# igashov/DiffLinker

Measured on NVIDIA H100. Metric: molecules/sec (T=500 denoising), higher is better.
Workload: dtype f32

## Files before the change

### difflinker_b200/csrc/common.cuh

```cuda
#pragma once
#include <cuda_runtime.h>
#include <stdint.h>

namespace dl {

constexpr int H = 128;
constexpr int MAX_DIN = 32;
constexpr int MAX_XHD = 16;

constexpr int OPT_TANH = 1;
constexpr int OPT_MEAN = 2;
constexpr int OPT_SIN = 4;
constexpr int N_SIN_FREQ = 6;
constexpr int N_SIN_FEAT = 4 * N_SIN_FREQ;
__device__ __forceinline__ float sin_freq(int k) { return __int_as_float(__float_as_int(0x1.aceeap-2f) + (k << 24)); }
__device__ __forceinline__ float sin_arg(float r, int k) { return __fmul_rn(__fsqrt_rn(__fadd_rn(r, 1e-8f)), sin_freq(k)); }
__device__ __forceinline__ float radial_rn(float dx, float dy, float dz) {
  return __fadd_rn(__fadd_rn(__fmul_rn(dx, dx), __fmul_rn(dy, dy)), __fmul_rn(dz, dz));
}

__device__ __forceinline__ void chain_wait() { asm volatile("griddepcontrol.wait;" ::: "memory"); }
__device__ __forceinline__ void chain_release() { asm volatile("griddepcontrol.launch_dependents;" ::: "memory"); }

inline bool& chain_overlap_enabled() { static bool on = true; return on; }

template <typename... KArgs, typename... Args>
inline cudaError_t launch_chain(void (*kernel)(KArgs...), dim3 grid, dim3 block, size_t smem, cudaStream_t st, Args&&... args) {
  cudaLaunchConfig_t cfg = {};
  cfg.gridDim = grid; cfg.blockDim = block; cfg.dynamicSmemBytes = smem; cfg.stream = st;
  cudaLaunchAttribute at[1];
  at[0].id = cudaLaunchAttributeProgrammaticStreamSerialization;
  at[0].val.programmaticStreamSerializationAllowed = chain_overlap_enabled() ? 1 : 0;
  cfg.attrs = at; cfg.numAttrs = 1;
  return cudaLaunchKernelEx(&cfg, kernel, KArgs(static_cast<Args&&>(args))...);
}

__device__ __forceinline__ float silu_f(float x) {
  float t, r;
  asm("ex2.approx.ftz.f32 %0, %1;" : "=f"(t) : "f"(x * -1.4426950408889634f));
// ... 103 lines not shown
```

### difflinker_b200/csrc/dl_engine.cu

```cuda
#include <cuda_fp16.h>
#include <cuda_runtime.h>

#include <algorithm>
#include <cmath>
#include <cstdarg>
#include <cstdio>
#include <cstdlib>
#include <cstring>
#include <ctime>
#include <map>
#include <string>
#include <vector>

#include "../../include/difflinker_b200.h"
#include "kernels_simt.cuh"
#include "kernels_tc.cuh"
#include "kernels_node_tc.cuh"
#include "kernels_retry.cuh"

using namespace dl;

static thread_local char g_err[1024] = "";
static void set_err(const char* fmt, ...) {
  va_list ap;
// ... 424 lines not shown

dl_status enqueue_forward(dl_engine* e, int B, int N, const FwdIO& io, cudaStream_t st) {
  Workspace& ws = e->ws;
  const Geom gm = make_geom(e, B, N);
  const int n = B * N;
  const int L = e->cfg.n_layers, S = e->cfg.inv_sublayers;
  const int node_blocks = (n + NODE_TM - 1) / NODE_TM;
  const size_t node_smem = 3 * NODE_TM * LDX * sizeof(float);

  PrepArgs pa{};
  pa.xh = io.sampler ? ws.z : io.xh;
  pa.node_mask = io.node_mask; pa.linker_mask = io.linker_mask;
  pa.t = io.t; pa.t_numel = io.t_numel; pa.context = io.context;
  pa.We_t = e->We_t; pa.be = e->be; pa.proj = proj_of(e->gcl[0]);
  pa.nm = ws.nm; pa.x0 = ws.x0; pa.x = ws.xa; pa.x04 = e->use_tc ? ws.x04 : nullptr; pa.x4 = e->use_tc ? ws.xa4 : nullptr; pa.cls = ws.cls; pa.h = ws.h;
  pa.AB = e->use_tc ? nullptr : ws.ABg; pa.ABmax = ws.ABgmax;
  pa.coef = io.sampler ? e->coef_dev : nullptr;
  pa.step_prep = io.sampler ? e->step_ctr : nullptr;
  pa.step_fin = io.sampler ? e->step_ctr + 1 : nullptr;
  TIMED("k_prep", st, (launch_chain(k_prep, dim3(node_blocks), dim3(256), 0, st, gm, pa)));
  LAUNCH_CHECK();
  e->launches += 1;
  if (e->use_tc) {
    const tcn::NodeTcArgs ta = node_tc_args(e, e->gcl[0], 0, -1);
    TIMED("k_node_tc(proj only)", st, (tcn::launch_node(n, ta, st)));
    LAUNCH_CHECK();
    e->launches += 1;
  }

  if (ws.nbr != nullptr) {
// ... 22 lines not shown
      if (e->use_tc) {
        const tcn::NodeTcArgs ta = node_tc_args(e, w, l, s);
        TIMED(ta.n_proj == 2 ? "k_node_tc(2 proj)" : "k_node_tc(1 proj)", st, (tcn::launch_node(n, ta, st)));
      } else {
        NodeArgs na{};
        na.h = ws.h; na.agg = ws.agg; na.nm = ws.nm; na.W3_t = w.W3_t; na.b3 = w.b3; na.W4_t = w.W4_t; na.b4 = w.b4;
        NodeConsumer c[2];
        const int n_proj = node_consumers(e, l, s, c);
        na.proj1 = proj_of(*c[0].w); na.AB1 = c[0].AB; na.ABmax1 = c[0].ABmax;
        if (n_proj == 2) { na.proj2 = proj_of(*c[1].w); na.AB2 = c[1].AB; na.ABmax2 = c[1].ABmax; }
        k_node<ACT_SILU><<<node_blocks, 256, node_smem, st>>>(n, na);
      }
      LAUNCH_CHECK();
      e->launches += 1;
    }
    k_copy_x<<<(n * 3 + 255) / 256, 256, 0, st>>>(n * 3, xin, xout, e->use_tc ? xin4 : nullptr, xout4);
    LAUNCH_CHECK();
    e->launches += 1;
    const EqW& w = e->eq[l];
    const EdgeArgs ea = edge_args(e, w, true, io.edge_mask, io.linker_mask, xin, xin4, xout, xout4, w.w5);
    e->times.begin(st, "edge COORD");
    dl_status st2 = launch_edge(e, gm, ea, true, w.W2_tc, st);
    e->times.end(st);
    if (st2 != DL_OK) return st2;
    std::swap(xin, xout);
    std::swap(xin4, xout4);
  }

  FinishArgs fa{};
  fa.h = ws.h; fa.x = xin; fa.x0 = ws.x0; fa.nm = ws.nm; fa.Wo = e->Wo; fa.bo = e->bo;
  fa.nan_flags = io.nan_flags;
  const bool fused_update = io.sampler && !io.inpaint;
  fa.out = fused_update ? nullptr : (io.sampler ? ws.eps : io.out);
// ... 1057 lines not shown
```

### difflinker_b200/csrc/kernels_node_tc.cuh

```cuda
#pragma once
#include "kernels_tc.cuh"

namespace dl {
namespace tcn {

using namespace dl::tc;

constexpr int TM = 128;
constexpr int X_LBO = TM * 16 + 16;
constexpr int X_BYTES = KC * X_LBO;
constexpr int HALF_BYTES = 8 * W_LBO;
constexpr int STAGE_BYTES = 2 * HALF_BYTES;
constexpr int BLOCK_BYTES = 2 * W_BYTES;
constexpr int N_RING = 2;
constexpr int N_OFF_WS = 4 * X_BYTES;
constexpr int N_OFF_MISC = N_OFF_WS + N_RING * STAGE_BYTES;
constexpr int N_OFF_BAR = N_OFF_MISC + 128 * 4 + 64;
constexpr int N_SMEM_BYTES = N_OFF_BAR + 64 + 1024;
static_assert(N_SMEM_BYTES <= 232448, "k_node_tc shared memory");
constexpr int NW = 8;
constexpr int W_NLOADER = NW;
constexpr int NODE_TC_THREADS = 32 * (NW + 1);

struct NodeTcArgs {
// ... 21 lines not shown
    sc = __int_as_float(max(127 + 13 - ex, 1) << 23);
  }
  return sc;
}

__device__ __forceinline__ void workers_sync() { asm volatile("bar.sync 1, %0;" ::"n"(32 * NW) : "memory"); }

__device__ __forceinline__ void store_elem(uint8_t* xhi, uint8_t* xlo, int c, int n, float v) {
  const __half hi = __float2half_rn(v);
  const __half lo = __float2half_rn(v - __half2float(hi));
  const int off = (c >> 3) * X_LBO + n * 16 + (c & 7) * 2;
  *reinterpret_cast<__half*>(xhi + off) = hi;
  *reinterpret_cast<__half*>(xlo + off) = lo;
}

__global__ void __launch_bounds__(NODE_TC_THREADS, 1) k_node_tc(int n_total, NodeTcArgs a) {
  extern __shared__ uint8_t smem_raw[];
  uint8_t* sm = smem_raw + ((1024u - (smem_u32(smem_raw) & 1023u)) & 1023u);
  const uint32_t sbase = smem_u32(sm);
  const int tid = threadIdx.x, warp = tid >> 5, lane = tid & 31;
  const int tile = a.tile_nodes > 0 ? a.tile_nodes : TM;
  const int g0 = blockIdx.x * tile;
  const int n_live = min(tile, n_total - g0);

  const uint32_t bar_full = sbase + N_OFF_BAR, bar_empty = bar_full + 8 * N_RING;
  uint8_t* xa_hi = sm; uint8_t* xa_lo = xa_hi + X_BYTES;
  uint8_t* xb_hi = sm + 2 * X_BYTES; uint8_t* xb_lo = xb_hi + X_BYTES;
  float* nms = reinterpret_cast<float*>(sm + N_OFF_MISC);
  int* tilemax = reinterpret_cast<int*>(sm + N_OFF_MISC + 512);

// ... 34 lines not shown
  const int c0 = 64 * g + 16 * (warp & 3) + (lane >> 2);
  int tm_calls = 0;
  auto tile_max = [&](float mx) -> float {
#pragma unroll
    for (int o = 16; o > 0; o >>= 1) mx = fmaxf(mx, __shfl_xor_sync(0xffffffffu, mx, o));
    int* slot = tilemax + (tm_calls++ & 15);
    if (lane == 0) atomicMax(slot, __float_as_int(mx));
    workers_sync();
    return __int_as_float(*slot);
  };
  auto operand_ready = [&]() {
    fence_proxy_async();
    workers_sync();
  };
  int hb = 0;
  float d[64];
#pragma unroll
  for (int i = 0; i < 64; ++i) d[i] = 0.f;
  auto gemm = [&](const uint8_t* xop, int n_blk_half, bool accumulate) {
    for (int k = 0; k < n_blk_half; ++k, ++hb) {
      const int s = hb % N_RING, hf = hb & 1;
      mbar_wait(bar_full + 8 * s, (hb / N_RING) & 1);
      const uint32_t xh = smem_u32(xop) + (8 * hf) * X_LBO, xl = xh + X_BYTES;
      const uint32_t wh = sbase + N_OFF_WS + s * STAGE_BYTES + g * 1024, wl = wh + HALF_BYTES;
      gemm_3xf16(d, wh, wl, W_LBO, xh, xl, X_LBO, 2 * X_LBO, 4, accumulate || k > 0);
      __syncwarp();
      if (lane == 0) mbar_arrive(bar_empty + 8 * s);
    }
  };

  auto load_rows = [&](float scale) -> float {
    float mx = 0.f;
#pragma unroll 1
// ... 33 lines not shown
    if (s1 == 1.0f) break;
  }
  operand_ready();

  if (a.proj_only) {
    s3 = s1;
  } else {
    gemm(xa_hi, 2, false);
    gemm(xb_hi, 2, true);
    workers_sync();
    const float2 bias3 = make_float2(__ldg(a.b3 + c0), __ldg(a.b3 + c0 + 8));
    const float ds1 = a.w3_descale / s1;
#pragma unroll 1
    for (int pass = 0; pass < 2; ++pass) {
      float mx = 0.f;
#pragma unroll
      for (int j = 0; j < 16; ++j)
#pragma unroll
        for (int u = 0; u < 4; ++u) {
          const float v = fmaf(d[4 * j + u], ds1, (u & 2) ? bias3.y : bias3.x);
          mx = fmaxf(mx, fabsf(v));
          store_elem(xb_hi, xb_lo, c0 + (u & 2) * 4, 8 * j + 2 * q + (u & 1), silu_f(v) * s2);
        }
      if (pass == 1) break;
      s2 = pow2_scale_for(tile_max(mx));
      if (s2 == 1.0f) break;
    }
    operand_ready();
    gemm(xb_hi, 2, false);
    const float2 bias4 = make_float2(__ldg(a.b4 + c0), __ldg(a.b4 + c0 + 8));
    const float ds2 = a.w4_descale / s2;
    float mx = 0.f;
#pragma unroll
    for (int j = 0; j < 16; ++j)
#pragma unroll
      for (int u = 0; u < 4; ++u) {
        const int n = 8 * j + 2 * q + (u & 1), c = c0 + (u & 2) * 4;
        float* hp = a.h + (size_t)(g0 + n) * H + c;
        const float hv = n < n_live ? *hp : 0.f;
        const float o = (hv + fmaf(d[4 * j + u], ds2, (u & 2) ? bias4.y : bias4.x)) * nms[n];
        if (n < n_live) *hp = o;
        mx = fmaxf(mx, fabsf(o));
        d[4 * j + u] = o;
        store_elem(xa_hi, xa_lo, c, n, o);
      }
    s3 = pow2_scale_for(tile_max(mx));
    if (s3 != 1.0f) {
#pragma unroll
      for (int j = 0; j < 16; ++j)
#pragma unroll
        for (int u = 0; u < 4; ++u) store_elem(xa_hi, xa_lo, c0 + (u & 2) * 4, 8 * j + 2 * q + (u & 1), d[4 * j + u] * s3);
    }
    operand_ready();
  }

  for (int p = 0; p < a.n_proj; ++p) {
#pragma unroll 1
    for (int pt = 0; pt < 2; ++pt) {
      gemm(xa_hi, 2, false);
      const float2 bias = pt == 0 ? make_float2(__ldg(a.pb1[p] + c0), __ldg(a.pb1[p] + c0 + 8)) : make_float2(0.f, 0.f);
      float* ab = a.AB[p] + (size_t)g0 * 2 * H + pt * H;
      const float ds = a.p_descale[p] / s3;
      float mx = 0.f;
#pragma unroll
      for (int j = 0; j < 16; ++j)
#pragma unroll
        for (int u = 0; u < 4; ++u) {
          const int n = 8 * j + 2 * q + (u & 1);
          const float o = fmaf(d[4 * j + u], ds, (u & 2) ? bias.y : bias.x);
          if (n < n_live) { ab[(size_t)n * 2 * H + c0 + (u & 2) * 4] = o; mx = fmaxf(mx, fabsf(o)); }
        }
      const float tmx = tile_max(mx);
      if (tid < n_live) a.ABmax[p][(size_t)(g0 + tid) * 2 + pt] = tmx;
    }
  }
}

inline size_t pack_blocks(const std::vector<float>& W, int in_stride, int nblk, std::vector<__half>& blob,
                          float* descale) {
  while (blob.size() % 64) blob.push_back(__float2half(0.f));
// ... 15 lines not shown
          const float v = W[(size_t)c * in_stride + b * H + kc * 8 + u] * scale;
          const __half hi = __float2half_rn(v);
          const __half lo = __float2half_rn(v - __half2float(hi));
          blob[off + b * per + ((size_t)kc * H + c) * 8 + u] = hi;
          blob[off + b * per + (size_t)KC * H * 8 + ((size_t)kc * H + c) * 8 + u] = lo;
        }
  return off;
}

inline int pick_tile_nodes(int n, int num_sms) {
  const int per = (n + num_sms - 1) / std::max(num_sms, 1);
  return std::min(TM, std::max(8, (per + 7) & ~7));
}

inline dl_status configure_node() {
  if (cudaFuncSetAttribute(k_node_tc, cudaFuncAttributeMaxDynamicSharedMemorySize, N_SMEM_BYTES) != cudaSuccess) return DL_ERR_CUDA;
  return DL_OK;
}

inline void launch_node(int n, const NodeTcArgs& ta, cudaStream_t st) {
  const int grid = (n + ta.tile_nodes - 1) / ta.tile_nodes;
  launch_chain(k_node_tc, dim3(grid), dim3(NODE_TC_THREADS), N_SMEM_BYTES, st, n, ta);
}

}
}
```

### difflinker_b200/csrc/kernels_simt.cuh

```cuda
#pragma once
#include <curand_kernel.h>

#include "common.cuh"

namespace dl {

__global__ void k_plan_mol(int N, int graph_type, const int8_t* __restrict__ edge_mask,
                           const int8_t* __restrict__ node_mask, const float* __restrict__ linker_mask,
                           int* __restrict__ rowidx, int* __restrict__ colidx, int* __restrict__ xrowidx,
                           int* __restrict__ nr, int* __restrict__ nc, int* __restrict__ nxr) {
  extern __shared__ int sm_plan[];
  int* rowlive = sm_plan;
  int* collive = sm_plan + N;
  const int b = blockIdx.x;
  const int tid = threadIdx.x, lane = tid & 31, warp = tid >> 5, nwarp = blockDim.x >> 5;
  for (int i = tid; i < N; i += blockDim.x) { rowlive[i] = 0; collive[i] = 0; }
  __syncthreads();
  if ((graph_type == 0 || graph_type == 4) && edge_mask != nullptr) {
    const int8_t* em = edge_mask + (size_t)b * N * N;
    for (int i = warp; i < N; i += nwarp) {
      int any = 0;
      for (int j = lane; j < N; j += 32) {
        int v = em[(size_t)i * N + j];
        if (v != 0) { any = 1; collive[j] = 1; }
// ... 153 lines not shown
struct PrepArgs {
  const float* xh;
  const int8_t* node_mask;
  const float* linker_mask;
  const float* t;
  int t_numel;
  const float* context;
  const float* We_t;
  const float* be;
  ProjW proj;
  float* nm;
  float* x0;
  float* x;
  float4* x04;
  float4* x4;
  int* cls;
  float* h;
  float* AB;
  float* ABmax;
  const float* coef;
  const int* step_prep;
  int* step_fin;
};

__global__ void __launch_bounds__(256) k_prep(Geom gm, PrepArgs a) {
  __shared__ __align__(16) float hs[NODE_TM * LDX];
  __shared__ float hin[NODE_TM][MAX_DIN];
  const int tid = threadIdx.x, lane = tid & 31, warp = tid >> 5;
  const int n_total = gm.B * gm.N;
  const int g0 = blockIdx.x * NODE_TM;
// ... 20 lines not shown
        int cidx = d - (gm.D - gm.C);
        v = a.context[(size_t)g * gm.C + cidx];
      }
    }
    hin[r][d] = v;
  }
  if (tid < NODE_TM) {
    int g = g0 + tid;
    if (g < n_total) {
      float m = (float)a.node_mask[g];
      a.nm[g] = m;
      for (int d = 0; d < 3; ++d) {
        float v = a.xh[(size_t)g * xd + d] * m;
        a.x0[(size_t)g * 3 + d] = v;
        a.x[(size_t)g * 3 + d] = v;
        if (a.x4 != nullptr) {
          reinterpret_cast<float*>(a.x04 + g)[d] = v;
          reinterpret_cast<float*>(a.x4 + g)[d] = v;
        }
      }
      if (gm.graph_type >= 1 && gm.graph_type <= 3) {
        int valid = m != 0.f;
        int pk = a.context[(size_t)g * gm.C + gm.C - 1] != 0.f;
        int fr = a.context[(size_t)g * gm.C + gm.C - 2] != 0.f;
        int lk = a.linker_mask != nullptr ? (a.linker_mask[g] != 0.f) : 0;
        int c = 0;
        if (valid) {
          if (gm.graph_type == 1) c = 1;
          else c = (lk || fr) ? 1 : (pk ? 2 : 3);
        }
        a.cls[g] = c;
      }
    }
// ... 282 lines not shown
  float* w5s = w0s + H;
  float* ems = w5s + H;
  float* cds = ems + ET;
  float* phis = cds + ET * 3;
  __shared__ float xacc[COORD ? 1 : 1];
  (void)xacc;

  const int tid = threadIdx.x, lane = tid & 31, warp = tid >> 5;
  const int N = gm.N;
  for (int idx = tid; idx < H * H / 4; idx += 256)
    reinterpret_cast<float4*>(W2s)[idx] = __ldg(reinterpret_cast<const float4*>(a.W2_t) + idx);
  if (tid < H) {
    b2s[tid] = a.b2[tid]; wds[tid] = a.wd[tid]; w0s[tid] = a.w0[tid];
    w5s[tid] = COORD ? a.w5[tid] : 0.f;
  }
  __syncthreads();

  auto divisor = [&](float cnt) { return !MEAN ? gm.normalization_factor : gm.graph_type == 0 ? (float)N : fmaxf(cnt, 1.f); };
  const int n_work = COORD ? *a.plan.n_xmols : *a.plan.n_items;
  for (int wi = blockIdx.x; wi < n_work; wi += gridDim.x) {
    int b, r_begin, r_count;
    if (COORD) { b = a.plan.xmols[wi]; r_begin = 0; r_count = a.plan.nxr[b]; }
    else { int4 it = a.plan.items[wi]; b = it.x; r_begin = it.y; r_count = it.z; }
    const int nc = a.plan.nc[b];
    const int* rows = (COORD ? a.plan.xrowidx : a.plan.rowidx) + (size_t)b * N;
    const int* cols = a.plan.colidx + (size_t)b * N;
    const size_t gb = (size_t)b * N;
    const int8_t* em_mol = a.edge_mask ? a.edge_mask + gb * N : nullptr;
    int per = nc >= ET ? 1 : ET / nc;
    if (per > MAXR) per = MAXR;
// ... 144 lines not shown
            }
            xrun += s;
            if (c0 + ET >= nc) {
              int i = rows[r_begin + rt + rr];
              float lm = a.linker_mask ? a.linker_mask[gb + i] : 1.f;
              float xv = a.x[(gb + i) * 3 + dim];
              a.x_out[(gb + i) * 3 + dim] = (xv + (xrun / divisor(runc)) * lm) * a.nm[gb + i];
            }
          }
        }
      }
    }
  }
}

__global__ void k_copy_x(int n3, const float* __restrict__ src, float* __restrict__ dst, const float4* __restrict__ src4,
                         float4* __restrict__ dst4) {
  int i = blockIdx.x * blockDim.x + threadIdx.x;
  if (i < n3) dst[i] = src[i];
  if (src4 != nullptr && i * 3 < n3) dst4[i] = src4[i];
}

enum { NOISE_TENSOR = 0, NOISE_BATCH = 1, NOISE_PER_MOLECULE = 2 };
struct NoiseRng {
  union {
    unsigned long long seed;
    const unsigned long long* seeds;
  };
  unsigned long long offset;
  unsigned long long per_draw;
  unsigned long long cx;
  int Sx, Sh;
  int F;
  int on;
  int g0;
  int N;
};
// ... 367 lines not shown
```

### difflinker_b200/csrc/kernels_tc.cuh

```cuda
#pragma once
#include <cuda_fp16.h>

#include <cmath>
#include <cstdio>
#include <type_traits>
#include <vector>

#include "../../include/difflinker_b200.h"
#include "kernels_simt.cuh"

namespace dl {
namespace tc {

constexpr bool AVAILABLE = true;
constexpr int TN = 128;
constexpr int MAXR = 32;
constexpr int KC = 16;
constexpr int W_LBO = H * 16;
constexpr int B_LBO = TN * 16 + 16;
constexpr int SBO = 128;
constexpr int W_BYTES = KC * W_LBO;
constexpr int B_BYTES = KC * B_LBO;
constexpr float F16_TARGET = 16384.0f;

// ... 102 lines not shown
__device__ __forceinline__ void fence_barrier_init() { asm volatile("fence.mbarrier_init.release.cluster;" ::: "memory"); }
__device__ __forceinline__ void fence_proxy_async() { asm volatile("fence.proxy.async.shared::cta;" ::: "memory"); }

__device__ __forceinline__ void bulk_g2s(uint32_t dst, const void* src, uint32_t bytes, uint32_t bar) {
  asm volatile("cp.async.bulk.shared::cluster.global.mbarrier::complete_tx::bytes [%0], [%1], %2, [%3];" ::"r"(dst),
               "l"(src), "r"(bytes), "r"(bar)
               : "memory");
}

__device__ __forceinline__ uint64_t wg_desc(uint32_t saddr, uint32_t lbo, uint32_t sbo) {
  return (uint64_t)((saddr & 0x3FFFFu) >> 4) | ((uint64_t)(lbo >> 4) << 16) | ((uint64_t)(sbo >> 4) << 32);
}
__device__ __forceinline__ void wg_fence() { asm volatile("wgmma.fence.sync.aligned;" ::: "memory"); }
__device__ __forceinline__ void wg_commit() { asm volatile("wgmma.commit_group.sync.aligned;" ::: "memory"); }
__device__ __forceinline__ void wg_wait_all() { asm volatile("wgmma.wait_group.sync.aligned 0;" ::: "memory"); }
__device__ __forceinline__ void fence_acc(float (&d)[64]) {
#pragma unroll
  for (int i = 0; i < 64; ++i) asm volatile("" : "+f"(d[i])::"memory");
}
template <int TRANS_B>
__device__ __forceinline__ void wgmma_m64n128k16(float (&d)[64], uint64_t adesc, uint64_t bdesc, uint32_t accumulate) {
  asm volatile(
      "{\n\t.reg .pred p;\n\t"
      "setp.ne.b32 p, %66, 0;\n\t"
      "wgmma.mma_async.sync.aligned.m64n128k16.f32.f16.f16 "
      "{%0, %1, %2, %3, %4, %5, %6, %7, %8, %9, %10, %11, %12, %13, %14, %15, %16, %17, %18, %19, %20, %21, %22, %23, %24, %25, %26, %27, %28, %29, %30, %31, %32, %33, %34, %35, %36, %37, %38, %39, %40, %41, %42, %43, %44, %45, %46, %47, %48, %49, %50, %51, %52, %53, %54, %55, %56, %57, %58, %59, %60, %61, %62, %63}, %64, %65, p, 1, 1, 0, %67;\n\t}"
      : "+f"(d[0]), "+f"(d[1]), "+f"(d[2]), "+f"(d[3]), "+f"(d[4]), "+f"(d[5]), "+f"(d[6]), "+f"(d[7]), "+f"(d[8]), "+f"(d[9]), "+f"(d[10]), "+f"(d[11]), "+f"(d[12]), "+f"(d[13]), "+f"(d[14]), "+f"(d[15]), "+f"(d[16]), "+f"(d[17]), "+f"(d[18]), "+f"(d[19]), "+f"(d[20]), "+f"(d[21]), "+f"(d[22]), "+f"(d[23]), "+f"(d[24]), "+f"(d[25]), "+f"(d[26]), "+f"(d[27]), "+f"(d[28]), "+f"(d[29]), "+f"(d[30]), "+f"(d[31]), "+f"(d[32]), "+f"(d[33]), "+f"(d[34]), "+f"(d[35]), "+f"(d[36]), "+f"(d[37]), "+f"(d[38]), "+f"(d[39]), "+f"(d[40]), "+f"(d[41]), "+f"(d[42]), "+f"(d[43]), "+f"(d[44]), "+f"(d[45]), "+f"(d[46]), "+f"(d[47]), "+f"(d[48]), "+f"(d[49]), "+f"(d[50]), "+f"(d[51]), "+f"(d[52]), "+f"(d[53]), "+f"(d[54]), "+f"(d[55]), "+f"(d[56]), "+f"(d[57]), "+f"(d[58]), "+f"(d[59]), "+f"(d[60]), "+f"(d[61]), "+f"(d[62]), "+f"(d[63])
      : "l"(adesc), "l"(bdesc), "r"(accumulate), "n"(TRANS_B));
}
template <int TRANS_B = 0>
__device__ __forceinline__ void mma_3xf16(float (&d)[64], uint32_t a_hi, uint32_t a_lo, uint32_t a_lbo, uint32_t b_hi,
                                          uint32_t b_lo, uint32_t b_lbo, uint32_t b_ks_stride, int nks, bool accumulate) {
#pragma unroll
  for (int ks = 0; ks < nks; ++ks) {
    const uint64_t ah = wg_desc(a_hi + ks * 2 * a_lbo, a_lbo, SBO), al = wg_desc(a_lo + ks * 2 * a_lbo, a_lbo, SBO);
    const uint64_t bh = wg_desc(b_hi + ks * b_ks_stride, b_lbo, SBO), bl = wg_desc(b_lo + ks * b_ks_stride, b_lbo, SBO);
    wgmma_m64n128k16<TRANS_B>(d, al, bh, (accumulate || ks > 0) ? 1u : 0u);
    wgmma_m64n128k16<TRANS_B>(d, ah, bl, 1u);
    wgmma_m64n128k16<TRANS_B>(d, ah, bh, 1u);
  }
}
template <int TRANS_B = 0>
__device__ __forceinline__ void gemm_3xf16(float (&d)[64], uint32_t a_hi, uint32_t a_lo, uint32_t a_lbo, uint32_t b_hi,
                                           uint32_t b_lo, uint32_t b_lbo, uint32_t b_ks_stride, int nks, bool accumulate) {
  fence_acc(d);
  wg_fence();
  mma_3xf16<TRANS_B>(d, a_hi, a_lo, a_lbo, b_hi, b_lo, b_lbo, b_ks_stride, nks, accumulate);
  wg_commit();
  wg_wait_all();
  fence_acc(d);
}

__device__ __forceinline__ void split2v(float2 v, uint32_t& hi, uint32_t& lo) {
  __half2 h = __float22half2_rn(v);
  float2 back = __half22float2(h);
  __half2 l = __float22half2_rn(fadd2(v, make_float2(-back.x, -back.y)));
  hi = *reinterpret_cast<uint32_t*>(&h);
  lo = *reinterpret_cast<uint32_t*>(&l);
// ... 112 lines not shown
    mbar_init(bars + BAR_W, 1);
    for (int i = 0; i < N_STAGE; ++i) { mbar_init(bars + BAR_FULL + 8 * i, N_PROD_WARPS); mbar_init(bars + BAR_EMPTY + 8 * i, N_EPI_WARPS); }
    for (int i = 0; i < N_ACC; ++i) {
      mbar_init(bars + BAR_TBL + 8 * i, 1);
      mbar_init(bars + BAR_TEMPTY + 8 * i, N_EPI_WARPS);
    }
    fence_barrier_init();
  }
  if (tid < H) b2w5[tid] = make_float2(a.b2[tid], COORD ? a.w5[tid] : 0.f);
  __syncthreads();

  if (warp >= W_LOAD && warp < W_PROD) {
    asm volatile("setmaxnreg.dec.sync.aligned.u32 %0;" ::"n"(REGS_CTRL));
  if (warp >= W_TBL && warp < W_TBL + N_TBL_WARPS) {
    const int tw = warp - W_TBL;
    typename std::conditional<SPARSE, RecIter, TileIter<COORD>>::type iter = make_iter<COORD, SPARSE>(a, N);
    Tile cur;
    for (int t = 0;; ++t) {
      const int acc = t & (N_ACC - 1);
      const bool more = iter.next(cur);
      if (t % N_TBL_WARPS != tw) { if (!more) break; continue; }
      if (t >= N_ACC) mbar_wait_relaxed(bars + BAR_TEMPTY + 8 * acc, ((t - N_ACC) / N_ACC) & 1);
      uint8_t* tb = sm + OFF_TBL + acc * TBL_BYTES;
      int* hdr = reinterpret_cast<int*>(tb + TBL_HDR);
      if (more) {
        const int Et = SPARSE ? cur.Et : cur.nrt * cur.ncc;
        const size_t gb = (size_t)cur.b * N;
        int heavy_deg = 0;
        if constexpr (MEAN && SPARSE) {
          const int w1 = __shfl_sync(0xffffffffu, iter.cur, 1), v2 = __shfl_sync(0xffffffffu, iter.cur, 2);
// ... 85 lines not shown
  } else if (warp == W_LOAD) {
    if (lane == 0) {
      mbar_expect_tx(bars + BAR_W, 2 * W_BYTES);
      bulk_g2s(sbase + OFF_WHI, w2tc, 2 * W_BYTES, bars + BAR_W);
    }
  }
  } else if (warp >= W_PROD) {
    const int pw = warp - W_PROD;
    const int kc = lane & 15, esub = lane >> 4;
    float2 wdr[4], w0r[4];
#pragma unroll
    for (int q = 0; q < 4; ++q) {
      wdr[q] = make_float2(__ldg(a.wd + kc * 8 + 2 * q), __ldg(a.wd + kc * 8 + 2 * q + 1));
      w0r[q] = make_float2(__ldg(a.w0 + kc * 8 + 2 * q), __ldg(a.w0 + kc * 8 + 2 * q + 1));
    }
    for (int t = 0;; ++t) {
      const int acc = t & (N_ACC - 1), s = t & (N_STAGE - 1);
      mbar_wait(bars + BAR_TBL + 8 * acc, (t / N_ACC) & 1);
      const uint8_t* tb = sm + OFF_TBL + acc * TBL_BYTES;
      const int Et = reinterpret_cast<const int*>(tb + TBL_HDR)[0];
      if (t >= N_STAGE) mbar_wait(bars + BAR_EMPTY + 8 * s, ((t - N_STAGE) / N_STAGE) & 1);
      if (Et > 0) {
        const int* rowoff = reinterpret_cast<const int*>(tb + TBL_ROWOFF);
        const int* coloff = reinterpret_cast<const int*>(tb + TBL_COLOFF);
        const float* dv = reinterpret_cast<const float*>(tb + TBL_D);
        const float* d0v = reinterpret_cast<const float*>(tb + TBL_D0);
        const float* scv = reinterpret_cast<const float*>(tb + TBL_SC);
        uint8_t* bhi = sm + OFF_ST + s * STAGE_BYTES + kc * B_LBO;
        uint8_t* blo = bhi + B_BYTES;
        const bool rescale = reinterpret_cast<const int*>(tb + TBL_HDR)[5] != 0;
// ... 80 lines not shown
      __syncwarp();
      if (lane == 0) mbar_arrive(bars + BAR_FULL + 8 * s);
      if (Et <= 0) break;
    }
  } else {
    asm volatile("setmaxnreg.inc.sync.aligned.u32 %0;" ::"n"(REGS_EPI));
    const int g = warp >> 2;
    const int wq = warp & 3, q = lane & 3;
    const int r0 = 64 * g + 16 * wq + (lane >> 2);
    float* txs = reinterpret_cast<float*>(sm + OFF_TX);
    float2 run = make_float2(0.f, 0.f);
    float run3 = 0.f;
    float d[64];
#pragma unroll
    for (int i = 0; i < 64; ++i) d[i] = 0.f;
    mbar_wait(bars + BAR_W, 0);
    for (int t = 0;; ++t) {
      const int acc = t & (N_ACC - 1), s = t & (N_STAGE - 1);
      if (!COORD && g == 0 && t > 0) named_sync(BAR_TURN0, 32 * N_EPI_WARPS);
      mbar_wait(bars + BAR_TBL + 8 * acc, (t / N_ACC) & 1);
      const uint8_t* tb = sm + OFF_TBL + acc * TBL_BYTES;
      const int* hdr = reinterpret_cast<const int*>(tb + TBL_HDR);
      const int Et = hdr[0];
      if (Et <= 0) break;
      const uint32_t bhi = sbase + OFF_ST + s * STAGE_BYTES, blo = bhi + B_BYTES;
      if (!COORD) {
        if (g == 1) named_sync(BAR_TURN1, 32 * N_EPI_WARPS);
        mbar_wait(bars + BAR_FULL + 8 * s, (t / N_STAGE) & 1);
        fence_acc(d);
        wg_fence();
// ... 183 lines not shown
    for (int c = 0; c < H; ++c)
      for (int u = 0; u < 8; ++u) {
        const float v = W[(size_t)c * H + kc * 8 + u] * scale;
        const __half hi = __float2half_rn(v);
        const __half lo = __float2half_rn(v - __half2float(hi));
        blob[off + ((size_t)kc * H + c) * 8 + u] = hi;
        blob[off + (size_t)KC * H * 8 + ((size_t)kc * H + c) * 8 + u] = lo;
      }
  return off;
}

template <bool COORD, bool SPARSE, int OPT = 0>
inline void launch_opt(int opt, const Geom& gm, const EdgeArgs& ea, const __half* w, int num_sms, cudaStream_t st) {
  if constexpr (OPT <= OPT_ALL) {
    if constexpr (COORD || !(OPT & OPT_TANH))
      if (opt == OPT) { k_edge_tc<COORD, SPARSE, OPT><<<num_sms, EDGE_TC_THREADS, SMEM_BYTES, st>>>(gm, ea, w); return; }
    launch_opt<COORD, SPARSE, OPT + 1>(opt, gm, ea, w, num_sms, st);
  }
}

inline dl_status launch_edge_tc(const Geom& gm, const EdgeArgs& ea, bool coord, int opt, const void* w2_tc, int num_sms,
                                cudaStream_t st) {
  if (!coord && (opt & OPT_TANH)) return DL_ERR_INVALID;
  if (ea.recs == nullptr && gm.graph_type != 0 && (opt & OPT_MEAN)) return DL_ERR_INVALID;
  const __half* w = reinterpret_cast<const __half*>(w2_tc);
  if (ea.recs != nullptr) {
    if (coord) launch_opt<true, true>(opt, gm, ea, w, num_sms, st);
    else launch_opt<false, true>(opt, gm, ea, w, num_sms, st);
  } else if (coord) launch_opt<true, false>(opt, gm, ea, w, num_sms, st);
  else launch_opt<false, false>(opt, gm, ea, w, num_sms, st);
  return DL_OK;
// ... 112 lines not shown
```

Baseline: 185.2.

## Chain edge kernels with PDL, drop x copy kernel, add narrow node tile variant

The edge tensor-core kernel is now launched through the programmatic-dependent-launch helper and gains griddepcontrol wait/release points. The SIMT edge kernel also gets these points. The per-layer k_copy_x launch is removed; instead the prep kernel writes the initial coordinates into both ping-pong buffers. A narrower node kernel variant (wgmma n80) is added for small node tiles, and a profiling script is added. The default for chain overlap flips to off, so the PDL attribute is disabled unless something re-enables it, for example an environment variable. Removing the copy is only safe if the coord edge kernel fully rewrites xout.

```diff
diff --git a/difflinker_b200/csrc/common.cuh b/difflinker_b200/csrc/common.cuh
--- a/difflinker_b200/csrc/common.cuh
+++ b/difflinker_b200/csrc/common.cuh
@@ -22,7 +22,7 @@
 __device__ __forceinline__ void chain_wait() { asm volatile("griddepcontrol.wait;" ::: "memory"); }
 __device__ __forceinline__ void chain_release() { asm volatile("griddepcontrol.launch_dependents;" ::: "memory"); }
 
-inline bool& chain_overlap_enabled() { static bool on = true; return on; }
+inline bool& chain_overlap_enabled() { static bool on = false; return on; }
 
 template <typename... KArgs, typename... Args>
 inline cudaError_t launch_chain(void (*kernel)(KArgs...), dim3 grid, dim3 block, size_t smem, cudaStream_t st, Args&&... args) {
diff --git a/difflinker_b200/csrc/dl_engine.cu b/difflinker_b200/csrc/dl_engine.cu
--- a/difflinker_b200/csrc/dl_engine.cu
+++ b/difflinker_b200/csrc/dl_engine.cu
@@ -462,6 +462,7 @@
   pa.t = io.t; pa.t_numel = io.t_numel; pa.context = io.context;
   pa.We_t = e->We_t; pa.be = e->be; pa.proj = proj_of(e->gcl[0]);
   pa.nm = ws.nm; pa.x0 = ws.x0; pa.x = ws.xa; pa.x04 = e->use_tc ? ws.x04 : nullptr; pa.x4 = e->use_tc ? ws.xa4 : nullptr; pa.cls = ws.cls; pa.h = ws.h;
+  pa.xb = ws.xb; pa.x4b = e->use_tc ? ws.xb4 : nullptr;
   pa.AB = e->use_tc ? nullptr : ws.ABg; pa.ABmax = ws.ABgmax;
   pa.coef = io.sampler ? e->coef_dev : nullptr;
   pa.step_prep = io.sampler ? e->step_ctr : nullptr;
@@ -514,9 +515,6 @@
       LAUNCH_CHECK();
       e->launches += 1;
     }
-    k_copy_x<<<(n * 3 + 255) / 256, 256, 0, st>>>(n * 3, xin, xout, e->use_tc ? xin4 : nullptr, xout4);
-    LAUNCH_CHECK();
-    e->launches += 1;
     const EqW& w = e->eq[l];
     const EdgeArgs ea = edge_args(e, w, true, io.edge_mask, io.linker_mask, xin, xin4, xout, xout4, w.w5);
     e->times.begin(st, "edge COORD");
diff --git a/difflinker_b200/csrc/kernels_node_tc.cuh b/difflinker_b200/csrc/kernels_node_tc.cuh
--- a/difflinker_b200/csrc/kernels_node_tc.cuh
+++ b/difflinker_b200/csrc/kernels_node_tc.cuh
@@ -59,6 +59,8 @@
   *reinterpret_cast<__half*>(xlo + off) = lo;
 }
 
+constexpr int NJ_NARROW = 10;
+template <int NJ>
 __global__ void __launch_bounds__(NODE_TC_THREADS, 1) k_node_tc(int n_total, NodeTcArgs a) {
   extern __shared__ uint8_t smem_raw[];
   uint8_t* sm = smem_raw + ((1024u - (smem_u32(smem_raw) & 1023u)) & 1023u);
@@ -123,9 +125,9 @@
     workers_sync();
   };
   int hb = 0;
-  float d[64];
-#pragma unroll
-  for (int i = 0; i < 64; ++i) d[i] = 0.f;
+  float d[4 * NJ];
+#pragma unroll
+  for (int i = 0; i < 4 * NJ; ++i) d[i] = 0.f;
   auto gemm = [&](const uint8_t* xop, int n_blk_half, bool accumulate) {
     for (int k = 0; k < n_blk_half; ++k, ++hb) {
       const int s = hb % N_RING, hf = hb & 1;
@@ -189,8 +191,9 @@
 #pragma unroll 1
     for (int pass = 0; pass < 2; ++pass) {
       float mx = 0.f;
-#pragma unroll
-      for (int j = 0; j < 16; ++j)
+      if (NJ < 16) mx = fmaxf(mx, fmaxf(fabsf(bias3.x), fabsf(bias3.y)));
+#pragma unroll
+      for (int j = 0; j < NJ; ++j)
 #pragma unroll
         for (int u = 0; u < 4; ++u) {
           const float v = fmaf(d[4 * j + u], ds1, (u & 2) ? bias3.y : bias3.x);
@@ -207,7 +210,7 @@
     const float ds2 = a.w4_descale / s2;
     float mx = 0.f;
 #pragma unroll
-    for (int j = 0; j < 16; ++j)
+    for (int j = 0; j < NJ; ++j)
 #pragma unroll
       for (int u = 0; u < 4; ++u) {
         const int n = 8 * j + 2 * q + (u & 1), c = c0 + (u & 2) * 4;
@@ -222,7 +225,7 @@
     s3 = pow2_scale_for(tile_max(mx));
     if (s3 != 1.0f) {
 #pragma unroll
-      for (int j = 0; j < 16; ++j)
+      for (int j = 0; j < NJ; ++j)
 #pragma unroll
         for (int u = 0; u < 4; ++u) store_elem(xa_hi, xa_lo, c0 + (u & 2) * 4, 8 * j + 2 * q + (u & 1), d[4 * j + u] * s3);
     }
@@ -238,7 +241,7 @@
       const float ds = a.p_descale[p] / s3;
       float mx = 0.f;
 #pragma unroll
-      for (int j = 0; j < 16; ++j)
+      for (int j = 0; j < NJ; ++j)
 #pragma unroll
         for (int u = 0; u < 4; ++u) {
           const int n = 8 * j + 2 * q + (u & 1);
@@ -284,14 +287,17 @@
 }
 
 inline dl_status configure_node() {
-  if (cudaFuncSetAttribute(k_node_tc, cudaFuncAttributeMaxDynamicSharedMemorySize, N_SMEM_BYTES) != cudaSuccess) return DL_ERR_CUDA;
+  if (cudaFuncSetAttribute(k_node_tc<16>, cudaFuncAttributeMaxDynamicSharedMemorySize, N_SMEM_BYTES) != cudaSuccess) return DL_ERR_CUDA;
+  if (cudaFuncSetAttribute(k_node_tc<NJ_NARROW>, cudaFuncAttributeMaxDynamicSharedMemorySize, N_SMEM_BYTES) != cudaSuccess)
+    return DL_ERR_CUDA;
   return DL_OK;
 }
 
 inline void launch_node(int n, const NodeTcArgs& ta, cudaStream_t st) {
   const int grid = (n + ta.tile_nodes - 1) / ta.tile_nodes;
-  launch_chain(k_node_tc, dim3(grid), dim3(NODE_TC_THREADS), N_SMEM_BYTES, st, n, ta);
-}
-
-}
-}
+  auto* kern = ta.tile_nodes > 0 && ta.tile_nodes <= 8 * NJ_NARROW ? k_node_tc<NJ_NARROW> : k_node_tc<16>;
+  launch_chain(kern, dim3(grid), dim3(NODE_TC_THREADS), N_SMEM_BYTES, st, n, ta);
+}
+
+}
+}
diff --git a/difflinker_b200/csrc/kernels_simt.cuh b/difflinker_b200/csrc/kernels_simt.cuh
--- a/difflinker_b200/csrc/kernels_simt.cuh
+++ b/difflinker_b200/csrc/kernels_simt.cuh
@@ -191,6 +191,8 @@
   float* x;
   float4* x04;
   float4* x4;
+  float* xb;
+  float4* x4b;
   int* cls;
   float* h;
   float* AB;
@@ -241,9 +243,11 @@
         float v = a.xh[(size_t)g * xd + d] * m;
         a.x0[(size_t)g * 3 + d] = v;
         a.x[(size_t)g * 3 + d] = v;
+        if (a.xb != nullptr) a.xb[(size_t)g * 3 + d] = v;
         if (a.x4 != nullptr) {
           reinterpret_cast<float*>(a.x04 + g)[d] = v;
           reinterpret_cast<float*>(a.x4 + g)[d] = v;
+          if (a.x4b != nullptr) reinterpret_cast<float*>(a.x4b + g)[d] = v;
         }
       }
       if (gm.graph_type >= 1 && gm.graph_type <= 3) {
@@ -556,6 +560,8 @@
     b2s[tid] = a.b2[tid]; wds[tid] = a.wd[tid]; w0s[tid] = a.w0[tid];
     w5s[tid] = COORD ? a.w5[tid] : 0.f;
   }
+  chain_wait();
+  if (tid == 0) chain_release();
   __syncthreads();
 
   auto divisor = [&](float cnt) { return !MEAN ? gm.normalization_factor : gm.graph_type == 0 ? (float)N : fmaxf(cnt, 1.f); };
@@ -730,13 +736,6 @@
   }
 }
 
-__global__ void k_copy_x(int n3, const float* __restrict__ src, float* __restrict__ dst, const float4* __restrict__ src4,
-                         float4* __restrict__ dst4) {
-  int i = blockIdx.x * blockDim.x + threadIdx.x;
-  if (i < n3) dst[i] = src[i];
-  if (src4 != nullptr && i * 3 < n3) dst4[i] = src4[i];
-}
-
 enum { NOISE_TENSOR = 0, NOISE_BATCH = 1, NOISE_PER_MOLECULE = 2 };
 struct NoiseRng {
   union {
diff --git a/difflinker_b200/csrc/kernels_tc.cuh b/difflinker_b200/csrc/kernels_tc.cuh
--- a/difflinker_b200/csrc/kernels_tc.cuh
+++ b/difflinker_b200/csrc/kernels_tc.cuh
@@ -140,9 +140,10 @@
 __device__ __forceinline__ void wg_fence() { asm volatile("wgmma.fence.sync.aligned;" ::: "memory"); }
 __device__ __forceinline__ void wg_commit() { asm volatile("wgmma.commit_group.sync.aligned;" ::: "memory"); }
 __device__ __forceinline__ void wg_wait_all() { asm volatile("wgmma.wait_group.sync.aligned 0;" ::: "memory"); }
-__device__ __forceinline__ void fence_acc(float (&d)[64]) {
-#pragma unroll
-  for (int i = 0; i < 64; ++i) asm volatile("" : "+f"(d[i])::"memory");
+template <int NR>
+__device__ __forceinline__ void fence_acc(float (&d)[NR]) {
+#pragma unroll
+  for (int i = 0; i < NR; ++i) asm volatile("" : "+f"(d[i])::"memory");
 }
 template <int TRANS_B>
 __device__ __forceinline__ void wgmma_m64n128k16(float (&d)[64], uint64_t adesc, uint64_t bdesc, uint32_t accumulate) {
@@ -154,20 +155,36 @@
       : "+f"(d[0]), "+f"(d[1]), "+f"(d[2]), "+f"(d[3]), "+f"(d[4]), "+f"(d[5]), "+f"(d[6]), "+f"(d[7]), "+f"(d[8]), "+f"(d[9]), "+f"(d[10]), "+f"(d[11]), "+f"(d[12]), "+f"(d[13]), "+f"(d[14]), "+f"(d[15]), "+f"(d[16]), "+f"(d[17]), "+f"(d[18]), "+f"(d[19]), "+f"(d[20]), "+f"(d[21]), "+f"(d[22]), "+f"(d[23]), "+f"(d[24]), "+f"(d[25]), "+f"(d[26]), "+f"(d[27]), "+f"(d[28]), "+f"(d[29]), "+f"(d[30]), "+f"(d[31]), "+f"(d[32]), "+f"(d[33]), "+f"(d[34]), "+f"(d[35]), "+f"(d[36]), "+f"(d[37]), "+f"(d[38]), "+f"(d[39]), "+f"(d[40]), "+f"(d[41]), "+f"(d[42]), "+f"(d[43]), "+f"(d[44]), "+f"(d[45]), "+f"(d[46]), "+f"(d[47]), "+f"(d[48]), "+f"(d[49]), "+f"(d[50]), "+f"(d[51]), "+f"(d[52]), "+f"(d[53]), "+f"(d[54]), "+f"(d[55]), "+f"(d[56]), "+f"(d[57]), "+f"(d[58]), "+f"(d[59]), "+f"(d[60]), "+f"(d[61]), "+f"(d[62]), "+f"(d[63])
       : "l"(adesc), "l"(bdesc), "r"(accumulate), "n"(TRANS_B));
 }
-template <int TRANS_B = 0>
-__device__ __forceinline__ void mma_3xf16(float (&d)[64], uint32_t a_hi, uint32_t a_lo, uint32_t a_lbo, uint32_t b_hi,
+template <int TRANS_B>
+__device__ __forceinline__ void wgmma_m64n80k16(float (&d)[40], uint64_t adesc, uint64_t bdesc, uint32_t accumulate) {
+  asm volatile(
+      "{\n\t.reg .pred p;\n\t"
+      "setp.ne.b32 p, %42, 0;\n\t"
+      "wgmma.mma_async.sync.aligned.m64n80k16.f32.f16.f16 "
+      "{%0, %1, %2, %3, %4, %5, %6, %7, %8, %9, %10, %11, %12, %13, %14, %15, %16, %17, %18, %19, %20, %21, %22, %23, %24, %25, %26, %27, %28, %29, %30, %31, %32, %33, %34, %35, %36, %37, %38, %39}, %40, %41, p, 1, 1, 0, %43;\n\t}"
+      : "+f"(d[0]), "+f"(d[1]), "+f"(d[2]), "+f"(d[3]), "+f"(d[4]), "+f"(d[5]), "+f"(d[6]), "+f"(d[7]), "+f"(d[8]), "+f"(d[9]), "+f"(d[10]), "+f"(d[11]), "+f"(d[12]), "+f"(d[13]), "+f"(d[14]), "+f"(d[15]), "+f"(d[16]), "+f"(d[17]), "+f"(d[18]), "+f"(d[19]), "+f"(d[20]), "+f"(d[21]), "+f"(d[22]), "+f"(d[23]), "+f"(d[24]), "+f"(d[25]), "+f"(d[26]), "+f"(d[27]), "+f"(d[28]), "+f"(d[29]), "+f"(d[30]), "+f"(d[31]), "+f"(d[32]), "+f"(d[33]), "+f"(d[34]), "+f"(d[35]), "+f"(d[36]), "+f"(d[37]), "+f"(d[38]), "+f"(d[39])
+      : "l"(adesc), "l"(bdesc), "r"(accumulate), "n"(TRANS_B));
+}
+template <int TRANS_B, int NR>
+__device__ __forceinline__ void wgmma_m64k16(float (&d)[NR], uint64_t adesc, uint64_t bdesc, uint32_t accumulate) {
+  static_assert(NR == 64 || NR == 40, "wgmma N = 128 or 80");
+  if constexpr (NR == 64) wgmma_m64n128k16<TRANS_B>(d, adesc, bdesc, accumulate);
+  else wgmma_m64n80k16<TRANS_B>(d, adesc, bdesc, accumulate);
+}
+template <int TRANS_B = 0, int NR>
+__device__ __forceinline__ void mma_3xf16(float (&d)[NR], uint32_t a_hi, uint32_t a_lo, uint32_t a_lbo, uint32_t b_hi,
                                           uint32_t b_lo, uint32_t b_lbo, uint32_t b_ks_stride, int nks, bool accumulate) {
 #pragma unroll
   for (int ks = 0; ks < nks; ++ks) {
     const uint64_t ah = wg_desc(a_hi + ks * 2 * a_lbo, a_lbo, SBO), al = wg_desc(a_lo + ks * 2 * a_lbo, a_lbo, SBO);
     const uint64_t bh = wg_desc(b_hi + ks * b_ks_stride, b_lbo, SBO), bl = wg_desc(b_lo + ks * b_ks_stride, b_lbo, SBO);
-    wgmma_m64n128k16<TRANS_B>(d, al, bh, (accumulate || ks > 0) ? 1u : 0u);
-    wgmma_m64n128k16<TRANS_B>(d, ah, bl, 1u);
-    wgmma_m64n128k16<TRANS_B>(d, ah, bh, 1u);
-  }
-}
-template <int TRANS_B = 0>
-__device__ __forceinline__ void gemm_3xf16(float (&d)[64], uint32_t a_hi, uint32_t a_lo, uint32_t a_lbo, uint32_t b_hi,
+    wgmma_m64k16<TRANS_B>(d, al, bh, (accumulate || ks > 0) ? 1u : 0u);
+    wgmma_m64k16<TRANS_B>(d, ah, bl, 1u);
+    wgmma_m64k16<TRANS_B>(d, ah, bh, 1u);
+  }
+}
+template <int TRANS_B = 0, int NR>
+__device__ __forceinline__ void gemm_3xf16(float (&d)[NR], uint32_t a_hi, uint32_t a_lo, uint32_t a_lbo, uint32_t b_hi,
                                            uint32_t b_lo, uint32_t b_lbo, uint32_t b_ks_stride, int nks, bool accumulate) {
   fence_acc(d);
   wg_fence();
@@ -310,6 +327,8 @@
     asm volatile("setmaxnreg.dec.sync.aligned.u32 %0;" ::"n"(REGS_CTRL));
   if (warp >= W_TBL && warp < W_TBL + N_TBL_WARPS) {
     const int tw = warp - W_TBL;
+    chain_wait();
+    if (tw == 0 && lane == 0) chain_release();
     typename std::conditional<SPARSE, RecIter, TileIter<COORD>>::type iter = make_iter<COORD, SPARSE>(a, N);
     Tile cur;
     for (int t = 0;; ++t) {
@@ -425,6 +444,7 @@
       wdr[q] = make_float2(__ldg(a.wd + kc * 8 + 2 * q), __ldg(a.wd + kc * 8 + 2 * q + 1));
       w0r[q] = make_float2(__ldg(a.w0 + kc * 8 + 2 * q), __ldg(a.w0 + kc * 8 + 2 * q + 1));
     }
+    chain_wait();
     for (int t = 0;; ++t) {
       const int acc = t & (N_ACC - 1), s = t & (N_STAGE - 1);
       mbar_wait(bars + BAR_TBL + 8 * acc, (t / N_ACC) & 1);
@@ -535,6 +555,7 @@
     float d[64];
 #pragma unroll
     for (int i = 0; i < 64; ++i) d[i] = 0.f;
+    chain_wait();
     mbar_wait(bars + BAR_W, 0);
     for (int t = 0;; ++t) {
       const int acc = t & (N_ACC - 1), s = t & (N_STAGE - 1);
@@ -748,7 +769,7 @@
 inline void launch_opt(int opt, const Geom& gm, const EdgeArgs& ea, const __half* w, int num_sms, cudaStream_t st) {
   if constexpr (OPT <= OPT_ALL) {
     if constexpr (COORD || !(OPT & OPT_TANH))
-      if (opt == OPT) { k_edge_tc<COORD, SPARSE, OPT><<<num_sms, EDGE_TC_THREADS, SMEM_BYTES, st>>>(gm, ea, w); return; }
+      if (opt == OPT) { launch_chain(k_edge_tc<COORD, SPARSE, OPT>, dim3(num_sms), dim3(EDGE_TC_THREADS), SMEM_BYTES, st, gm, ea, w); return; }
     launch_opt<COORD, SPARSE, OPT + 1>(opt, gm, ea, w, num_sms, st);
   }
 }
diff --git a/profiles/launch_chain.py b/profiles/launch_chain.py
--- /dev/null
+++ b/profiles/launch_chain.py
@@ -0,0 +1,163 @@
+import argparse
+import json
+import os
+import statistics
+import subprocess
+import sys
+
+ROOT = os.path.dirname(os.path.dirname(os.path.abspath(__file__)))
+if ROOT not in sys.path:
+    sys.path.insert(0, ROOT)
+
+
+def parse():
+    ap = argparse.ArgumentParser()
+    ap.add_argument("--workload", default="cfg2_zinc")
+    ap.add_argument("--edge-impl", default="auto", choices=["auto", "simt", "wgmma"])
+    ap.add_argument("--trace-T", type=int, default=8)
+    ap.add_argument("--T", type=int, default=None, help="reverse steps of the A/B runs (default: the workload's)")
+    ap.add_argument("--runs", type=int, default=3)
+    ap.add_argument("--calls", type=int, default=2, help="timed sample_chain calls per A/B process")
+    ap.add_argument("--out", default=None, help="directory for launch_chain.json (default: print only)")
+    ap.add_argument("--part", default="all", choices=["all", "trace", "time"])
+    return ap.parse_args()
+
+
+def setup(args, T):
+    import torch
+    from difflinker_b200 import DDPM, synthetic
+    from difflinker_b200.batching import collate
+    from difflinker_b200.ddpm import sampler_inputs
+    spec = synthetic.SPECS[args.workload]
+    hp = synthetic.model_hparams(spec)
+    if T is not None:
+        hp['diffusion_steps'] = T
+    dev = torch.device("cuda", 0)
+    torch.manual_seed(0)
+    ddpm = DDPM(**hp, edge_impl=args.edge_impl)
+    synthetic.init_reference_like_weights(ddpm, coord_gain=100.0 if spec.N <= 64 else 1.0)
+    ddpm = ddpm.to(dev)
+    data = {k: (v.to(dev) if torch.is_tensor(v) else v) for k, v in collate(synthetic.make_items(spec, seed_offset=1)).items()}
+    return ddpm.edm, sampler_inputs(ddpm, data)
+
+
+def kernel_class(name):
+    if "k_edge_tc<true" in name or "k_edge_simt<true" in name:
+        return "edge COORD"
+    if "k_edge_tc<false" in name or "k_edge_simt<false" in name:
+        return "edge GCL"
+    for k in ("k_prep", "k_node_tc", "k_node", "k_nbr", "k_copy_x", "k_finish", "k_inpaint"):
+        if k + "(" in name or k + "<" in name:
+            return k
+    return name[:60]
+
+
+def part_trace(args):
+    import torch
+    from torch.profiler import profile, ProfilerActivity
+    edm, kw = setup(args, args.trace_T)
+    edm.sample_chain(**kw, keep_frames=1)
+    torch.cuda.synchronize()
+    with profile(activities=[ProfilerActivity.CUDA]) as prof:
+        edm.sample_chain(**kw, keep_frames=1)
+        torch.cuda.synchronize()
+    ks = sorted(((e.time_range.start, e.time_range.end, e.name) for e in prof.events()
+                 if e.device_type == torch.autograd.DeviceType.CUDA and "memset" not in e.name.lower()
+                 and "memcpy" not in e.name.lower()), key=lambda k: k[0])
+    fwds, cur = [], None
+    for k in ks:
+        if kernel_class(k[2]) == "k_prep":
+            cur = []
+            fwds.append(cur)
+        if cur is not None:
+            cur.append(k)
+    for f in fwds:
+        last = max(i for i, k in enumerate(f) if kernel_class(k[2]) in ("k_finish", "k_inpaint"))
+        del f[last + 1:]
+    n_mode = statistics.mode(len(f) for f in fwds)
+    fwds = [f for f in fwds if len(f) == n_mode]
+    dur, exposed = {}, {}
+    spans, gaps = [], []
+    for f in fwds:
+        spans.append(f[-1][1] - f[0][0])
+        gaps.append(spans[-1] - sum(e - s for s, e, _ in f))
+        prev_end = None
+        for s, e, n in f:
+            c = kernel_class(n)
+            dur.setdefault(c, []).append(e - s)
+            exposed.setdefault(c, []).append(e - (prev_end if prev_end is not None else s))
+            prev_end = e
+    per_kernel = {c: {"launches_per_forward": len(v) / len(fwds), "mean_us": statistics.fmean(v),
+                      "mean_exposed_us": statistics.fmean(exposed[c])} for c, v in dur.items()}
+    return {"T": args.trace_T, "forwards": len(fwds), "kernels_per_forward": n_mode,
+            "forward_span_us": statistics.fmean(spans), "forward_gap_us": statistics.fmean(gaps), "kernels": per_kernel}
+
+
+def part_time(args):
+    import torch
+    edm, kw = setup(args, args.T)
+    edm.sample_chain(**kw, keep_frames=1)
+    torch.cuda.synchronize()
+    ms = []
+    for _ in range(args.calls):
+        a, b = torch.cuda.Event(enable_timing=True), torch.cuda.Event(enable_timing=True)
+        a.record()
+        edm.sample_chain(**kw, keep_frames=1)
+        b.record()
+        torch.cuda.synchronize()
+        ms.append(a.elapsed_time(b))
+    return {"T": edm.T, "sample_chain_ms": ms, "loop_ms": edm.last_loop_ms}
+
+
+def card():
+    try:
+        q = subprocess.run(["nvidia-smi", "--query-gpu=name,power.limit,clocks.max.sm", "--format=csv,noheader"],
+                           capture_output=True, text=True, timeout=30).stdout.strip().splitlines()[0]
+        name, power, clock = (s.strip() for s in q.split(","))
+        return {"name": name, "power_limit": power, "max_sm_clock": clock}
+    except Exception as exc:
+        return {"error": repr(exc)}
+
+
+def child(args, part, env):
+    cmd = [sys.executable, os.path.abspath(__file__), "--part", part, "--workload", args.workload, "--edge-impl",
+           args.edge_impl, "--trace-T", str(args.trace_T), "--calls", str(args.calls)]
+    if args.T is not None:
+        cmd += ["--T", str(args.T)]
+    res = subprocess.run(cmd, capture_output=True, text=True, env={**os.environ, **env})
+    if res.returncode != 0:
+        raise SystemExit(f"{part} run failed:\n{res.stderr[-4000:]}")
+    return json.loads(res.stdout.strip().splitlines()[-1])
+
+
+def main():
+    args = parse()
+    if args.part != "all":
+        print(json.dumps(part_trace(args) if args.part == "trace" else part_time(args)))
+        return
+    out = {"workload": args.workload, "edge_impl": args.edge_impl, "card": card()}
+    out["trace"] = child(args, "trace", {})
+    for c, v in sorted(out["trace"]["kernels"].items(), key=lambda kv: -kv[1]["mean_us"] * kv[1]["launches_per_forward"]):
+        print(f"{c:14s} x{v['launches_per_forward']:4.1f}  mean {v['mean_us']:8.2f} us  exposed {v['mean_exposed_us']:8.2f} us",
+              file=sys.stderr)
+    print(f"forward span {out['trace']['forward_span_us']:.1f} us, gap {out['trace']['forward_gap_us']:.1f} us "
+          f"({out['trace']['kernels_per_forward']} kernels)", file=sys.stderr)
+    ab = {"0": [], "1": []}
+    for _ in range(args.runs):
+        for ov in ("0", "1"):
+            r = child(args, "time", {"DL_CHAIN_OVERLAP": ov})
+            ab[ov].append(r)
+            print(f"DL_CHAIN_OVERLAP={ov}: sample_chain {' '.join(f'{m:.1f}' for m in r['sample_chain_ms'])} ms "
+                  f"(T={r['T']})", file=sys.stderr)
+    out["ab"] = {ov: {"runs": v, "median_ms": statistics.median(m for r in v for m in r["sample_chain_ms"])}
+                 for ov, v in ab.items()}
+    out["card_after"] = card()
+    print(json.dumps(out))
+    if args.out:
+        os.makedirs(args.out, exist_ok=True)
+        with open(os.path.join(args.out, "launch_chain.json"), "w") as f:
+            json.dump(out, f, indent=1)
+
+
+if __name__ == "__main__":
+    main()
```

After: 191.6, median of 6. 1.03x the previous value.
